# jinhojsk515/spmm

Measured on AMD Instinct MI355X. Metric: pretrain molecules/sec, higher is better.
Workload: dtype bf16; 1 GPU; SPMM pretrain step, text 12 layers (fusion at 6) + PV 6 layers, H=768, 12 heads, queue 36864, train mode (dropout 0.1), fwd+bwd+clip+AdamW+EMA; global_batch=128, seq_len=128, parallelism=dp1, schedule=eager launches on three HIP streams, packed text rows

## Files before the change

include/spmm_hip.h:

```cpp
#ifndef SPMM_HIP_H
#define SPMM_HIP_H

#include <stdint.h>

#ifdef __HIPCC__
#include <hip/hip_runtime.h>
typedef hipStream_t spmm_stream_t;
#else
typedef void* spmm_stream_t;
#endif

#ifdef __cplusplus
extern "C" {
#endif

int spmm_version(void);
const char* spmm_last_error(void);

#define SPMM_EPI_BF16 0
#define SPMM_EPI_GELU 1
#define SPMM_EPI_F32 2
#define SPMM_EPI_F32_ATOMIC 3
#define SPMM_EPI_GELU_GRAD 4
#define SPMM_EPI_F32_ACC 5
#define SPMM_EPI_GELU_DERIV 6
#define SPMM_EPI_MUL 7

#define SPMM_GEMM_AUTO 0
#define SPMM_GEMM_K128 1
#define SPMM_GEMM_K256x128 2
#define SPMM_GEMM_K256 3
#define SPMM_GEMM_K128PC 5
#define SPMM_GEMM_K256P8 8
#define SPMM_GEMM_K256P8_TILES 9
#define SPMM_GEMM_AUTO_TILES 16
int spmm_gemm_nt(const void* A, long lda, const void* W, long ldw, int M, int N, int K, int splits, const float* bias,
                 const float* div_ptr, float alpha, const void* R, long ldr, const void* G, long ldg, void* C, long ldc,
                 void* C2, long ldc2, int epi, float* colsum, int kernel, const int* M_dev, spmm_stream_t stream);
long spmm_gemm_tn_workspace_bytes(int M, int N, int K, int splits);
int spmm_gemm_tn_splits(int M, int N, int K, int kernel);
int spmm_gemm_tn(const void* A, long lda, const void* B, long ldb, int M, int N, int K, int splits, float alpha, float* C,
                 long ldc, float* workspace, int kernel, const int* M_dev, spmm_stream_t stream);
int spmm_gemm_tn_reduce(const float* ws, int ns, int N, int K, float* C, long ldc, spmm_stream_t stream);
int spmm_colsum_bf16(const void* x, long ld, int R, int C, float* out, const int* R_dev, spmm_stream_t stream);

int spmm_attn_fwd(const void* Q, long ldq, const void* K, long ldk, const void* V, long ldv, const int* kmask,
                  const int* kv_seq, const int* q_row0, const int* q_len, const int* kv_row0, const int* kv_len, void* O,
                  long ldo, float* LSE, int nseq, int nH, int Lq, int Lkv, int causal_from, int is_cross, float dropout_p,
                  const uint64_t* seed_ptr, uint64_t seed_salt, int q_off, int kv_off, spmm_stream_t stream);
int spmm_attn_bwd(const void* Q, long ldq, const void* K, long ldk, const void* V, long ldv, const int* kmask,
                  const int* kv_seq, const int* q_row0, const int* q_len, const int* kv_row0, const int* kv_len,
                  const void* O, long ldo, const float* LSE, const void* dO, long lddo, void* dQ,
                  long lddq, void* dK, long lddk, void* dV, long lddv, int nseq, int nH, int Lq, int Lkv, int causal_from,
                  int is_cross, float dropout_p, const uint64_t* seed_ptr, uint64_t seed_salt, int q_off, int kv_off, int d_mode,
                  float* Dbuf, spmm_stream_t stream);

int spmm_xattn_supported(int H, int nH, int Lq, int Lkv);
int spmm_xattn_pack_wo(const void* W, long ldw, void* out, int H, spmm_stream_t stream);
int spmm_xattn_fwd(const void* Q, long ldq, const void* K, long ldk, const void* V, long ldv, const int* kmask,
                   const int* kv_seq, const int* q_row0, const int* q_len, const int* kv_row0, const int* kv_len,
                   const void* WoF, const float* bo, const void* R, long ldr, const float* gamma, const float* beta, float eps,
                   void* Y, long ldy, void* Z, long ldz, float* mean, float* rstd, void* CTX, long ldc, float* LSE,
                   int nseq, int nH, int Lq, int Lkv, float attn_dropout_p, uint64_t salt_a, float hidden_dropout_p,
                   uint64_t salt_h, const uint64_t* seed_ptr, long row_base, spmm_stream_t stream);
int spmm_segment_sum_bf16(const void* src, const int* start, const int* list, void* out, int U, long W, spmm_stream_t stream);

int spmm_ln_fwd(const void* x, const void* res, const float* gamma, const float* beta, void* y, void* zout, float* mean,
                float* rstd, long rows, int H, float eps, float dropout_p, const uint64_t* seed_ptr, uint64_t salt,
                const int* rows_dev, spmm_stream_t stream);
int spmm_ln_fwd_r32(const void* x, const float* res32, const float* gamma, const float* beta, void* y, float* y32, void* zout,
                    float* mean, float* rstd, long rows, int H, float eps, float dropout_p, const uint64_t* seed_ptr,
// ... 90 lines not shown
```

spmm_amd/csrc/gemm.hip:

```cpp
#include "common.h"
#include "../../include/spmm_hip.h"

namespace {

constexpr int BM = 128, BN = 128, BK = 64;
constexpr int TILE_BYTES = BM * BK * 2;
constexpr int STAGE_BYTES = 2 * TILE_BYTES;

enum Epi { EPI_BF16 = 0, EPI_GELU = 1, EPI_F32 = 2, EPI_F32_ATOMIC = 3, EPI_GELU_GRAD = 4, EPI_F32_ACC = 5, EPI_GELU_DERIV = 6, EPI_MUL = 7 };
constexpr bool epi_is_bf16(int e) { return e == EPI_BF16 || e == EPI_GELU || e == EPI_GELU_GRAD || e == EPI_GELU_DERIV || e == EPI_MUL; }

struct GemmP {
  const bf16* A; long lda;
  const bf16* W; long ldw;
  int M, N, K;
  int ksplit;
  const float* bias;
  const float* div_ptr;
  float alpha;
  const bf16* R; long ldr;
  const bf16* G; long ldg;
  void* C; long ldc;
  bf16* C2; long ldc2;
  float* colsum;
  int order;
  const int* M_ptr;
};

#define GEMM_DYN_M(P)                                          \
  do {                                                         \
    if ((P).M_ptr) {                                           \
      const int m_ = *(P).M_ptr;                               \
      (P).M = m_ < (P).M ? (m_ > 0 ? m_ : 1) : (P).M;          \
    }                                                          \
  } while (0)

__device__ __forceinline__ void stage_tile_dma(const bf16* __restrict__ src, long ld, int row0, int nrows, int k0,
                                               char* lds_tile, int tid) {
#pragma unroll
  for (int c = 0; c < 4; ++c) {
    const int id = c * 256 + tid;
    const int row = id >> 3, ps = id & 7;
    const int ls = ps ^ ((row >> 1) & 7);
    int grow = row0 + row;
    grow = grow < nrows ? grow : nrows - 1;
    const bf16* g = src + (long)grow * ld + k0 + ls * 8;
    const int wave_base = __builtin_amdgcn_readfirstlane((c * 256 + (tid & ~63)) * 16);
    __builtin_amdgcn_global_load_lds((const GLOBAL_AS void*)g, (LDS_AS void*)(lds_tile + wave_base), 16, 0, 0);
  }
}

template <int EPI>
__device__ __forceinline__ void epi_convert(const GemmP& p, f32x16 (&acc)[2][2], char* t0, char* t1, int n_base, int lane) {
  float scale = p.alpha;
  if (p.div_ptr) scale /= *p.div_ptr;
#pragma unroll
  for (int ni = 0; ni < 2; ++ni)
#pragma unroll
    for (int mi = 0; mi < 2; ++mi) {
// ... 788 lines not shown
      if constexpr (HAS_EX && EPI == EPI_GELU_GRAD) {
        if (blk == 3) { P8_LOAD_EX(1); }
      } else if constexpr (HAS_EX) {
        if (h == 0) {
#pragma unroll
          for (int i_ = 2 * mi; i_ < 2 * mi + 2; ++i_) {
            long r_ = row0 + 64 + i_ * 8;
            if (!INTERIOR) r_ = r_ < p.M ? r_ : p.M - 1;
            P8_EX_LOAD1(i_, r_);
          }
        }
      }
    }
#undef P8_LOAD_EX
#undef P8_EX_LOAD1
  if constexpr (!GELU2) {
    if (p.colsum) {
#pragma unroll
      for (int e = 0; e < 8; ++e) {
        float t = cs[e];
        t += __shfl_xor(t, 8, 64);
        t += __shfl_xor(t, 16, 64);
        t += __shfl_xor(t, 32, 64);
        cs[e] = t;
      }
      if (lane < 8 && n_ok) {
#pragma unroll
        for (int e = 0; e < 8; ++e) atomicAdd(p.colsum + n + e, cs[e]);
      }
    }
  }
}

template <int EPI>
__global__ __launch_bounds__(512) void gemm_nt_p8_kernel(GemmP p) {
  extern __shared__ __attribute__((aligned(16))) char smem8[];
  const int tid = threadIdx.x, lane = tid & 63;
  const int wave = __builtin_amdgcn_readfirstlane(tid >> 6);
  const int wr = wave >> 2, wc = wave & 3;
  GEMM_DYN_M(p);
  const int ntm = (p.M + BM3 - 1) / BM3, ntn = (p.N + BN3 - 1) / BN3, nt = ntm * ntn;
  if ((int)blockIdx.x >= nt) return;
  const int nk = p.K / BK;

  f32x4 acc[2][4][4];
#define P8_ZERO()                                                              \
  _Pragma("unroll") for (int h_ = 0; h_ < 2; ++h_)                             \
  _Pragma("unroll") for (int i_ = 0; i_ < 4; ++i_)                             \
  _Pragma("unroll") for (int j_ = 0; j_ < 4; ++j_) acc[h_][i_][j_] = f32x4{0.f, 0.f, 0.f, 0.f}
  P8_ZERO();

  uint32_t offA[2][2], offW[2][2];
  const uint32_t ls16 = (uint32_t)(((tid & 7) ^ ((tid >> 4) & 7)) * 16);
  int m0, n0;
#define P8_TILE(VB)                                                                                           \
  do {                                                                                                        \
    const int b_ = (VB), q_ = nt >> 3, r_ = nt & 7, xcd_ = b_ & 7, i_ = b_ >> 3;                              \
    const int t_ = (xcd_ < r_ ? xcd_ * (q_ + 1) : r_ * (q_ + 1) + (xcd_ - r_) * q_) + i_;                     \
    int tm_, tn_;                                                                                             \
    tile_of(t_, ntm, ntn, p.order, tm_, tn_);                                                                 \
    m0 = tm_ * BM3; n0 = tn_ * BN3;                                                                           \
    _Pragma("unroll") for (int h_ = 0; h_ < 2; ++h_)                                                          \
    _Pragma("unroll") for (int j_ = 0; j_ < 2; ++j_) {                                                        \
      int row_ = m0 + j_ * 128 + h_ * 64 + (tid >> 3);                                                        \
      row_ = row_ < p.M ? row_ : p.M - 1;                     \
      offA[h_][j_] = (uint32_t)row_ * (uint32_t)(p.lda * 2) + ls16;                                                      \
      int col_ = n0 + (j_ * 2 + (tid >> 8)) * 64 + h_ * 32 + ((tid >> 3) & 31);                               \
      col_ = col_ < p.N ? col_ : p.N - 1;                                                                     \
      offW[h_][j_] = (uint32_t)col_ * (uint32_t)(p.ldw * 2) + ls16;                                                      \
    }                                                                                                         \
  } while (0)
  const char* gA = (const char*)p.A;
  const char* gW = (const char*)p.W;
  const uint32_t lds0 = (uint32_t)(uintptr_t)(LDS_AS char*)smem8;
#define P8_STG(GB, O, SLOT)                                                                                               \
  do {                                                                                                                    \
    const uint32_t d_ = lds0 + (SLOT) + wave * 1024;                                                                      \
    asm volatile("s_mov_b32 m0, %2\n\ts_nop 0\n\tglobal_load_lds_dwordx4 %0, %1" :: "v"((O)[0]), "s"(GB), "s"(d_) : "memory", "m0");          \
    asm volatile("s_mov_b32 m0, %2\n\ts_nop 0\n\tglobal_load_lds_dwordx4 %0, %1" :: "v"((O)[1]), "s"(GB), "s"(d_ + 8192) : "memory", "m0");   \
  } while (0)
#define P8_STG_A(H, BUF, KT) P8_STG((const char*)(gA + (size_t)(KT) * (BK * 2)), offA[H], (BUF) * P8_BUF + (H) * P8_HT)
#define P8_STG_W(H, BUF, KT) P8_STG((const char*)(gW + (size_t)(KT) * (BK * 2)), offW[H], (BUF) * P8_BUF + (2 + (H)) * P8_HT)
#define P8_PROLOGUE()                                                                        \
  do {                                                                                       \
    P8_STG_A(0, 0, 0); P8_STG_W(0, 0, 0); P8_STG_W(1, 0, 0); P8_STG_A(1, 0, 0);              \
    P8_STG_W(0, 1, 1); P8_STG_A(0, 1, 1); P8_STG_W(1, 1, 1);                                 \
  } while (0)

  uint32_t aad[2][2], wad[2][2];
  {
    const uint32_t sw = (uint32_t)((lane >> 1) & 7), r16 = (uint32_t)(lane & 15), q = (uint32_t)(lane >> 4);
#pragma unroll
    for (int kk = 0; kk < 2; ++kk) {
      const uint32_t slot = ((((uint32_t)kk * 4 + q) ^ sw) << 4);
      aad[0][kk] = lds0 + ((uint32_t)wr * 64 + r16) * 128 + slot;
      wad[0][kk] = lds0 + 2 * P8_HT + ((uint32_t)wc * 32 + r16) * 128 + slot;
      aad[1][kk] = aad[0][kk] + P8_BUF;
      wad[1][kk] = wad[0][kk] + P8_BUF;
    }
  }
  bf16x8 fa[4][2], fw0[2][2], fw1[2][2];
#define P8_RD_A(BUF, H)                                                                       \
// ... 27 lines not shown
#define P8_LGKM0() asm volatile("s_waitcnt lgkmcnt(0)" ::: "memory")
#define P8_COMPUTE(H, NH, FW)                    \
  do {                                           \
    P8_BAR();                                    \
    P8_LGKM0();                                  \
    P8_SB();                                     \
    __builtin_amdgcn_s_setprio(1);               \
    P8_MM(H, NH, FW);                            \
    __builtin_amdgcn_s_setprio(0);               \
    P8_SB();                                     \
    P8_BAR();                                    \
    P8_SB();                                     \
  } while (0)

#ifdef P8_PROFILE
  unsigned long long* prof = (unsigned long long*)p.colsum + (size_t)blockIdx.x * 16 * 8;
  p.colsum = nullptr;
  int prof_i = 0;
#define P8_STAMP(K) do { if (prof && tid == 0 && prof_i < 16) prof[prof_i * 8 + (K)] = __builtin_readcyclecounter(); } while (0)
#else
#define P8_STAMP(K) do { } while (0)
#endif
  int vb = blockIdx.x;
  bool pre = false;
  P8_TILE(vb);
  P8_PROLOGUE();
  asm volatile("s_waitcnt vmcnt(6)" ::: "memory");
  P8_BAR();
  P8_SB();
  if (wr == 1) P8_BAR();
  for (;;) {
    P8_STAMP(0);
    const int cm0 = m0, cn0 = n0;
    const int vbn = vb + (int)gridDim.x;
    const bool has_next = vbn < nt;
    const bool pre_next = has_next && cm0 + BM3 <= p.M && cn0 + BN3 <= p.N;
    for (int kt = 0; kt < nk; kt += 2) {
      const bool last = kt + 2 >= nk;
      const bool more = !last || has_next;
      int kn = kt + 2;
      P8_RD_W(0, 0, fw0); P8_SB(); P8_RD_A(0, 0);
      if (!(pre && kt == 0)) P8_STG_A(1, 1, kt + 1);
      asm volatile("s_waitcnt lgkmcnt(8)" ::: "memory");
      P8_COMPUTE(0, 0, fw0);
      if (last && has_next) { P8_TILE(vbn); kn = 0; }
      P8_RD_W(0, 1, fw1);
      if (more) P8_STG_W(0, 0, kn);
      P8_COMPUTE(0, 1, fw1);
      P8_RD_A(0, 1);
      if (more) P8_STG_A(0, 0, kn);
      P8_COMPUTE(1, 1, fw1);
      if (more) {
        P8_STG_W(1, 0, kn);
        if (pre && kt == 0) asm volatile("s_waitcnt vmcnt(22)" ::: "memory");
        else asm volatile("s_waitcnt vmcnt(6)" ::: "memory");
      } else {
        asm volatile("s_waitcnt vmcnt(0)" ::: "memory");
      }
      P8_COMPUTE(1, 0, fw0);
      P8_RD_W(1, 0, fw0); P8_SB(); P8_RD_A(1, 0);
      if (more) P8_STG_A(1, 0, kn);
      asm volatile("s_waitcnt lgkmcnt(8)" ::: "memory");
      P8_COMPUTE(0, 0, fw0);
      P8_RD_W(1, 1, fw1);
      if (more) P8_STG_W(0, 1, kn + 1);
      P8_COMPUTE(0, 1, fw1);
      P8_RD_A(1, 1);
      if (more) P8_STG_A(0, 1, kn + 1);
      P8_COMPUTE(1, 1, fw1);
      if (more) {
        P8_STG_W(1, 1, kn + 1);
        if (last && pre_next) {
          P8_STG_A(1, 1, kn + 1);
          asm volatile("s_waitcnt vmcnt(8)" ::: "memory");
        } else {
          asm volatile("s_waitcnt vmcnt(6)" ::: "memory");
        }
      }
      P8_COMPUTE(1, 0, fw0);
    }
    P8_STAMP(2);

    if (wr == 0) P8_BAR();
    P8_SB();
    {
      int lane_e = lane;
      asm volatile("" : "+v"(lane_e));
      GemmP q = p;
      asm volatile("" : "+s"(q.C), "+s"(q.ldc), "+s"(q.C2), "+s"(q.ldc2));
      asm volatile("" : "+s"(q.R), "+s"(q.ldr), "+s"(q.G), "+s"(q.ldg));
      asm volatile("" : "+s"(q.bias), "+s"(q.colsum), "+s"(q.div_ptr), "+s"(q.alpha), "+s"(q.M), "+s"(q.N));
      auto hook = [](int) {};
      const uint32_t xb = lds0 + P8_LDS + wave * 4096;
      const int mb = cm0 + wr * 128, nb = cn0 + wc * 64;
      const bool interior = cm0 + BM3 <= q.M && cn0 + BN3 <= q.N;
      if constexpr (EPI == EPI_GELU_GRAD || EPI == EPI_MUL) {
        if (interior) p8_epilogue_blocks<EPI, true, true>(q, acc, xb, mb, nb, lane_e, hook);
        else p8_epilogue_blocks<EPI, false, true>(q, acc, xb, mb, nb, lane_e, hook);
      } else if (EPI == EPI_BF16 && q.R != nullptr) {
        if (interior) p8_epilogue_blocks<EPI, true, true>(q, acc, xb, mb, nb, lane_e, hook);
        else p8_epilogue_blocks<EPI, false, true>(q, acc, xb, mb, nb, lane_e, hook);
      } else {
        if (interior) p8_epilogue_blocks<EPI, true, false>(q, acc, xb, mb, nb, lane_e, hook);
        else p8_epilogue_blocks<EPI, false, false>(q, acc, xb, mb, nb, lane_e, hook);
      }
    }
    P8_SB();
    if (wr == 1) P8_BAR();
    P8_STAMP(4);
#ifdef P8_PROFILE
    ++prof_i;
#endif
    if (!has_next) break;
    vb = vbn;
    pre = pre_next;
    P8_SB();
  }
  if (wr == 0) P8_BAR();
#undef P8_ZERO
#undef P8_STAMP
#undef P8_TILE
#undef P8_PROLOGUE
#undef P8_STG
#undef P8_STG_A
#undef P8_STG_W
#undef P8_RD_A
#undef P8_RD_W
#undef P8_MM
#undef P8_COMPUTE
#undef P8_BAR
#undef P8_SB
#undef P8_LGKM0
}

template <typename K>
int raise_lds(K kernel, int bytes, const char* what) {
  hipError_t e = hipFuncSetAttribute((const void*)kernel, hipFuncAttributeMaxDynamicSharedMemorySize, bytes);
  if (e != hipSuccess) {
    spmm_set_error("spmm_gemm_nt: cannot raise the dynamic LDS of %s to %d: %s", what, bytes, hipGetErrorString(e));
    return SPMM_ERR_LAUNCH;
  }
  return SPMM_OK;
}

template <int EPI>
int launch_p8_one(const GemmP& p, hipStream_t st, bool persist) {
  static const int rc = raise_lds(gemm_nt_p8_kernel<EPI>, P8_LDS + P8_XLDS, "the 8-phase kernel");
  if (rc != SPMM_OK) return rc;
  const int nt = ((p.M + BM3 - 1) / BM3) * ((p.N + BN3 - 1) / BN3);
  static const int ncu = [] { int dev = 0, n = 0; (void)hipGetDevice(&dev); (void)hipDeviceGetAttribute(&n, hipDeviceAttributeMultiprocessorCount, dev); return n > 0 ? n & ~7 : 256; }();
  dim3 grid(persist && nt > ncu ? ncu : nt);
  hipLaunchKernelGGL((gemm_nt_p8_kernel<EPI>), grid, dim3(512), P8_LDS + P8_XLDS, st, p);
  return SPMM_OK;
}
int launch_p8(int epi, const GemmP& p, hipStream_t st, bool persist) {
  switch (epi) {
    case EPI_BF16: return launch_p8_one<EPI_BF16>(p, st, persist);
    case EPI_GELU: return launch_p8_one<EPI_GELU>(p, st, persist);
    case EPI_GELU_GRAD: return launch_p8_one<EPI_GELU_GRAD>(p, st, persist);
    case EPI_GELU_DERIV: return launch_p8_one<EPI_GELU_DERIV>(p, st, persist);
    case EPI_MUL: return launch_p8_one<EPI_MUL>(p, st, persist);
    default: return -1;
  }
}

template <int EPI>
int launch_v3_one(const GemmP& p, hipStream_t st) {
  static const int rc = raise_lds(gemm_nt_v3_kernel<EPI>, LDS3_BYTES, "the 256x256 kernel");
  if (rc != SPMM_OK) return rc;
  dim3 grid(((p.M + BM3 - 1) / BM3) * ((p.N + BN3 - 1) / BN3));
  hipLaunchKernelGGL((gemm_nt_v3_kernel<EPI>), grid, dim3(512), LDS3_BYTES, st, p);
  return SPMM_OK;
}
int launch_v3(int epi, const GemmP& p, hipStream_t st) {
  switch (epi) {
    case EPI_BF16: return launch_v3_one<EPI_BF16>(p, st);
    case EPI_GELU: return launch_v3_one<EPI_GELU>(p, st);
    case EPI_GELU_GRAD: return launch_v3_one<EPI_GELU_GRAD>(p, st);
    case EPI_GELU_DERIV: return launch_v3_one<EPI_GELU_DERIV>(p, st);
    case EPI_MUL: return launch_v3_one<EPI_MUL>(p, st);
    default: return -1;
  }
}

// ... 46 lines not shown
    case EPI_F32_ATOMIC: hipLaunchKernelGGL((gemm_nt_kernel<EPI_F32_ATOMIC>), grid, dim3(256), 0, st, p); break;
    case EPI_GELU_GRAD: hipLaunchKernelGGL((gemm_nt_kernel<EPI_GELU_GRAD>), grid, dim3(256), 0, st, p); break;
    case EPI_F32_ACC: hipLaunchKernelGGL((gemm_nt_kernel<EPI_F32_ACC>), grid, dim3(256), 0, st, p); break;
    case EPI_GELU_DERIV: hipLaunchKernelGGL((gemm_nt_kernel<EPI_GELU_DERIV>), grid, dim3(256), 0, st, p); break;
    case EPI_MUL: hipLaunchKernelGGL((gemm_nt_kernel<EPI_MUL>), grid, dim3(256), 0, st, p); break;
    default: return -1;
  }
  return SPMM_OK;
}

inline bool is_bf16_epi(int epi) { return epi_is_bf16(epi); }
inline bool p8_ok(const GemmP& p, int epi) {
  return is_bf16_epi(epi) && p.K % 128 == 0 && p.N % 8 == 0 && (unsigned long)p.M * (unsigned long)p.lda * 2ul < (1ul << 32) &&
         (unsigned long)p.N * (unsigned long)p.ldw * 2ul < (1ul << 32);
}

int pick_tile(int M, int N, int epi) {
  const bool bf = is_bf16_epi(epi);
  if (M >= 6000) {
    const long t3 = (long)((M + 255) / 256) * ((N + 255) / 256);
    if (bf && t3 >= 96) return 3;
    return (epi != EPI_F32_ATOMIC) ? 2 : 1;
  }
  auto tiles = [&](int bm, int bn) { return (double)((M + bm - 1) / bm) * ((N + bn - 1) / bn); };
  auto fill = [](double t) { const double w = (double)(long)((t + 255) / 256); return t / (256.0 * w); };
  const double t3 = tiles(256, 256), t2 = tiles(256, 128), t1 = tiles(128, 128);
  const double s3 = bf ? 1.20 * fill(t3) : 0.0;
  const double s2 = (M >= 512 && epi != EPI_F32_ATOMIC) ? 0.85 * fill(t2) : 0.0;
  const double s1 = 0.80 * (t1 < 256 ? t1 / 256.0 : 1.0);
  if (s3 >= s2 && s3 >= s1) return 3;
  return s2 >= s1 ? 2 : 1;
}

}

extern "C" int spmm_gemm_nt(const void* A, long lda, const void* W, long ldw, int M, int N, int K, int splits,
                            const float* bias, const float* div_ptr, float alpha, const void* R, long ldr,
                            const void* G, long ldg, void* C, long ldc, void* C2, long ldc2, int epi, float* colsum,
                            int kernel, const int* M_dev, hipStream_t stream) {
  SPMM_CHECK_SHAPE(M > 0 && N > 0 && K > 0, "spmm_gemm_nt: empty problem M=%d N=%d K=%d", M, N, K);
  SPMM_CHECK_SHAPE(K % 64 == 0, "spmm_gemm_nt: K=%d must be a multiple of 64", K);
  SPMM_CHECK_SHAPE(N % 4 == 0, "spmm_gemm_nt: N=%d must be a multiple of 4", N);
  SPMM_CHECK_SHAPE(lda % 8 == 0 && ldw % 8 == 0, "spmm_gemm_nt: lda/ldw must be multiples of 8 elements");
  SPMM_CHECK_SHAPE(ldc % 4 == 0, "spmm_gemm_nt: ldc must be a multiple of 4");
  SPMM_CHECK_SHAPE(!is_bf16_epi(epi) || (ldc % 8 == 0 && (!R || ldr % 8 == 0) && (!G || ldg % 8 == 0) && (!C2 || ldc2 % 8 == 0) && (uintptr_t)C % 16 == 0),
                   "spmm_gemm_nt: bf16 outputs need 16-B aligned rows (ldc/ldr/ldg/ldc2 multiples of 8)");
  SPMM_CHECK_SHAPE(((uintptr_t)A % 16 == 0) && ((uintptr_t)W % 16 == 0), "spmm_gemm_nt: A/W must be 16-B aligned");
  SPMM_CHECK_SHAPE(epi >= EPI_BF16 && epi <= EPI_MUL, "spmm_gemm_nt: unknown epilogue %d", epi);
  if (splits < 1) splits = 1;
  SPMM_CHECK_SHAPE(splits == 1 || epi == EPI_F32_ATOMIC, "spmm_gemm_nt: split-K needs the atomic epilogue");
  SPMM_CHECK_SHAPE((epi != EPI_GELU_GRAD && epi != EPI_MUL) || G != nullptr, "spmm_gemm_nt: the GELU-grad / multiply epilogues need G");
  SPMM_CHECK_SHAPE(colsum == nullptr || epi == EPI_BF16 || epi == EPI_GELU_GRAD || epi == EPI_MUL, "spmm_gemm_nt: colsum is only fused into the bf16 / GELU-grad / multiply epilogues");
  int ksplit = ((K / 64 + splits - 1) / splits) * 64;
  splits = (K + ksplit - 1) / ksplit;
  GemmP p;
  p.A = (const bf16*)A; p.lda = lda; p.W = (const bf16*)W; p.ldw = ldw;
  p.M = M; p.N = N; p.K = K; p.ksplit = ksplit; p.bias = bias; p.div_ptr = div_ptr; p.alpha = alpha;
  p.R = (const bf16*)R; p.ldr = ldr; p.G = (const bf16*)G; p.ldg = ldg; p.C = C; p.ldc = ldc;
  p.C2 = (bf16*)C2; p.ldc2 = ldc2; p.colsum = colsum;
  p.M_ptr = nullptr;
  p.order = K > 1024 ? 0 : 2;

  int k = kernel == SPMM_GEMM_AUTO_TILES ? 0 : kernel;
  if (k == 0) {
    const int tile = splits > 1 ? 1 : pick_tile(M, N, epi);
    k = tile == 3 ? (p8_ok(p, epi) ? (kernel == SPMM_GEMM_AUTO_TILES ? 9 : 8) : 3) : tile;
    if (k == 2 && (epi == EPI_F32_ATOMIC || M < 512)) k = 1;
  }
  const bool pc_fits = (unsigned long)p.M * (unsigned long)p.lda * 2ul < (1ul << 32) && (unsigned long)p.N * (unsigned long)p.ldw * 2ul < (1ul << 32);
  const long t128 = (long)((M + BM - 1) / BM) * ((N + BN - 1) / BN) * splits;
  if (k == 1 && kernel != 1 && pc_fits && PC_AUTO && t128 <= 256 && ksplit >= 4 * BK) k = 5;
  SPMM_CHECK_SHAPE(k == 1 || k == 2 || k == 3 || k == 5 || k == 8 || k == 9, "spmm_gemm_nt: unknown kernel selector %d", kernel);
  SPMM_CHECK_SHAPE(k != 5 || pc_fits, "spmm_gemm_nt: kernel 5 addresses its operands with 32-bit byte offsets (< 4 GiB each)");
  SPMM_CHECK_SHAPE((k != 8 && k != 9) || p8_ok(p, epi), "spmm_gemm_nt: the 8-phase kernel needs a bf16-output epilogue, K %% 128 == 0, N %% 8 == 0 and operands < 4 GiB");
  SPMM_CHECK_SHAPE(k != 3 || is_bf16_epi(epi), "spmm_gemm_nt: the 256x256 kernel has bf16-output epilogues only");
  SPMM_CHECK_SHAPE(k != 2 || epi != EPI_F32_ATOMIC, "spmm_gemm_nt: the 256x128 kernel has no atomic epilogue");
  SPMM_CHECK_SHAPE(k == 1 || k == 5 || splits == 1, "spmm_gemm_nt: split-K runs on the 128x128 kernels only");
  p.M_ptr = M_dev;
  int rc;
  if (k == 8 || k == 9) rc = launch_p8(epi, p, stream, k == 8);
  else if (k == 3) rc = launch_v3(epi, p, stream);
  else if (k == 2) rc = launch_v2(epi, p, stream);
  else if (k == 5) rc = launch_pc(epi, p, dim3(((M + BM - 1) / BM) * ((N + BN - 1) / BN), 1, splits), stream);
  else rc = launch_v1(epi, p, dim3(((M + BM - 1) / BM) * ((N + BN - 1) / BN), 1, splits), stream);
  if (rc > 0) return rc;
  if (rc < 0) { spmm_set_error("spmm_gemm_nt: epilogue %d is not built for kernel %d", epi, k); return SPMM_ERR_UNSUPPORTED; }
  SPMM_LAUNCH_CHECK("spmm_gemm_nt");
  return SPMM_OK;
}
```

spmm_amd/engine.py:

```python
from __future__ import annotations

import contextlib
import functools
from dataclasses import dataclass
from typing import List, Optional

import torch

from . import ops, streams
from .config import BertConfig, SPMMConfig
from .options import EngineOptions
from .params import ParamStore

BF = torch.bfloat16
LOSS_MLM, LOSS_MPM, LOSS_ITA, LOSS_ITM = 0, 1, 2, 3


def _ceil(x, m):
    return (x + m - 1) // m * m


class KVSource:

    def __init__(self, kv: torch.Tensor, U: int, Lkv: int, row0=None, length=None, pack_idx=None):
# ... 60 lines not shown
        return self

    def attend(self, src: KVSource, idx: torch.Tensor) -> "Group":
        self.src, self.Lkv = src, src.Lkv
        self.kv_off = src.add(idx)
        self.kv_idx = idx.to(torch.int32)
        return self

    def cross_layout(self) -> dict:
        src = self.src
        return dict(kmask=self.kv_mask, kv_seq=self.kv_idx, q_row0=self.q_row0, q_len=self.q_len,
                    kv_row0=None if src is None else src.row0, kv_len=None if src is None else src.len)


@dataclass
class Batch:
    groups: List[Group]
    rows_dev: Optional[torch.Tensor] = None

    def __iter__(self):
        return iter(self.groups)

    def __len__(self):
        return len(self.groups)


STREAM_TOKENS_MAX = 49152


class Engine:
    def __init__(self, cfg: SPMMConfig, params: ParamStore, device, options: Optional[EngineOptions] = None):
        self.cfg, self.P, self.dev = cfg, params, device
        self.opt = options if options is not None else EngineOptions.from_env()
        if torch.device(device).type == "cuda":
            from ._lib import bind_device
            bind_device(torch.device(device).index if torch.device(device).index is not None else torch.cuda.current_device())
        f32 = dict(dtype=torch.float32, device=device)
        self.alpha = torch.zeros(1, **f32)
        self.lr = torch.zeros(1, **f32)
        self.gscale = torch.ones(4, **f32)
        self.step_zero = torch.zeros(16, dtype=torch.int32, device=device)
        self.losses = self.step_zero[0:8].view(torch.float32)
        self.loss_scratch = torch.zeros(8, **f32)
        rank = torch.distributed.get_rank() if (torch.distributed.is_available() and torch.distributed.is_initialized()) else 0
        self.seed_rank_offset = rank * 0x9E3779B97F4A7C15 % (1 << 62)
        self.seed = torch.full((1,), (0x5DEECE66D + self.seed_rank_offset) % (1 << 62), dtype=torch.int64, device=device)
        self.nan_flag = self.step_zero[9:10]
        self.icount = torch.zeros(4, dtype=torch.int32, device=device)
        self.dtemp_ita = self.step_zero[8:9].view(torch.float32)
        self.train_mode = True
        self.hint_bad = self.step_zero[10:11]
        self.pack_text = self.opt.pack_text
        self.layer_done_cb = None
        self.multi_stream = self.opt.multi_stream
        self.wgrad_async = self.opt.wgrad_stream and self.multi_stream
        self._one_stream = False
        dist_ = torch.distributed
        will_exchange = dist_.is_available() and dist_.is_initialized() and (dist_.get_world_size() > 1 or self.opt.force_dist)
        self._one_side = bool(will_exchange and self.opt.dp_four_streams)
        if self.multi_stream and torch.device(device).type == "cuda" and not ops._DRY_RUN and not will_exchange:
            streams.bind_in_order(device, ("side0", "side1", "wgrad"))
        self.force_one_stream = False
        self._wg_stream, self._wg_pending, self._wg_keep = None, False, []
        self._salt = 0
        self._off_path_ok, self._pre_bwd = False, None
        self._xattn_checked = self._xattn_off = False
# ... 497 lines not shown
```

spmm_amd/ops.py:

```python
import ctypes
import os

import torch

from ._lib import lib

EPI_BF16, EPI_GELU, EPI_F32, EPI_F32_ATOMIC, EPI_GELU_GRAD, EPI_F32_ACC, EPI_GELU_DERIV, EPI_MUL = range(8)
BF16 = torch.bfloat16


_DRY_RUN = False
_dry_log = []


def _p(t):
    return None if t is None else ctypes.c_void_p(t.data_ptr())


def _st():
    if _DRY_RUN:
        return None
    return ctypes.c_void_p(torch.cuda.current_stream().cuda_stream)


# ... 19 lines not shown
            raise TypeError(f"{name}: argument {i} = {a!r} is not a {t.__name__}") from e
        if t is ctypes.c_void_p and not (a is None or isinstance(a, (ctypes.c_void_p, int))):
            raise TypeError(f"{name}: argument {i} must be a pointer, got {type(a)}")
    _dry_log.append(name)


def _row_stride(t):
    assert t.dim() == 2 and (t.stride(1) == 1 or t.shape[1] == 1), (t.shape, t.stride())
    return t.stride(0)


GEMM_AUTO, GEMM_AUTO_TILES = 0, 16
_nt_auto = GEMM_AUTO


class nt_tiles_per_workgroup:

    def __init__(self, on=True):
        self.on = on

    def __enter__(self):
        global _nt_auto
        self._prev = _nt_auto
        if self.on:
            _nt_auto = GEMM_AUTO_TILES
        return self

    def __exit__(self, *exc):
        global _nt_auto
        _nt_auto = self._prev
        return False


def gemm_nt(A, W, C, *, bias=None, epi=EPI_BF16, R=None, G=None, C2=None, alpha=1.0, div=None, splits=1, K=None, colsum=None, kernel=0,
            M_dev=None):
    if kernel == 0:
        kernel = _nt_auto
    M, Ka = A.shape
    N = W.shape[0]
    K = Ka if K is None else K
    assert A.dtype == BF16 and W.dtype == BF16 and W.shape[1] >= K and C.shape[0] >= M and C.shape[1] >= N
    if epi in (EPI_BF16, EPI_GELU, EPI_GELU_GRAD, EPI_GELU_DERIV, EPI_MUL):
        assert C.dtype == BF16
    else:
        assert C.dtype == torch.float32
    _call("spmm_gemm_nt", _p(A), _row_stride(A), _p(W), _row_stride(W), M, N, K, splits, _p(bias), _p(div),
               float(alpha), _p(R), 0 if R is None else _row_stride(R), _p(G), 0 if G is None else _row_stride(G),
               _p(C), _row_stride(C), _p(C2), 0 if C2 is None else _row_stride(C2), epi, _p(colsum), int(kernel), _p(M_dev), _st())
    return C


def gemm_tn(A, B, C, *, alpha=1.0, splits=None, kernel=0, M_dev=None):
    M, N = A.shape
    K = B.shape[1]
    assert A.dtype == BF16 and B.dtype == BF16 and C.dtype == torch.float32 and B.shape[0] == M and tuple(C.shape) == (N, K)
    if splits is None:
        splits = 1 if _DRY_RUN else lib().cdll.spmm_gemm_tn_splits(M, N, K, int(kernel))
    ws = torch.empty(splits * N * K, dtype=torch.float32, device=C.device) if splits > 1 else None
    _call("spmm_gemm_tn", _p(A), _row_stride(A), _p(B), _row_stride(B), M, N, K, splits, float(alpha), _p(C), _row_stride(C), _p(ws),
          int(kernel), _p(M_dev), _st())
    return C


def colsum_bf16(x, out, *, R_dev=None):
    R, C = x.shape
    _call("spmm_colsum_bf16", _p(x), _row_stride(x), R, C, _p(out), _p(R_dev), _st())
    return out


def attn_fwd(Q, K, V, O, lse, *, nseq, nH, Lq, Lkv, kmask=None, causal_from=None, is_cross=False, dropout_p=0.0,
             seed=None, salt=0, kv_seq=None, q_row0=None, q_len=None, kv_row0=None, kv_len=None, q_off=0, kv_off=0):
    cf = nseq if causal_from is None else causal_from
    _call("spmm_attn_fwd", _p(Q), _row_stride(Q), _p(K), _row_stride(K), _p(V), _row_stride(V), _p(kmask), _p(kv_seq), _p(q_row0),
               _p(q_len), _p(kv_row0), _p(kv_len), _p(O),
               _row_stride(O), _p(lse), nseq, nH, Lq, Lkv, cf, int(is_cross), float(dropout_p), _p(seed), salt, int(q_off), int(kv_off), _st())
    return O


def attn_bwd(Q, K, V, O, lse, dO, dQ, dK, dV, *, nseq, nH, Lq, Lkv, kmask=None, causal_from=None, is_cross=False,
             dropout_p=0.0, seed=None, salt=0, kv_seq=None, q_row0=None, q_len=None, kv_row0=None, kv_len=None, q_off=0, kv_off=0,
             d_mode=0, dbuf=None):
# ... 434 lines not shown
```

spmm_amd/options.py:

```python
from __future__ import annotations

import dataclasses
import os
from dataclasses import dataclass

_ENV = {
    "pack_text": ("SPMM_PACK_TEXT", lambda s: s != "0"),
    "cls_only_top": ("SPMM_CLS_ONLY_TOP", lambda s: s != "0"),
    "multi_stream": ("SPMM_STREAMS", lambda s: s != "1"),
    "wgrad_stream": ("SPMM_WGRAD_STREAM", lambda s: s != "0"),
    "pv_wgrad_inline": ("SPMM_PV_WGRAD_INLINE", int),
    "ln_from_y": ("SPMM_LN_FROM_Y", lambda s: s != "0"),
    "resid_fp32": ("SPMM_RESID_FP32", lambda s: s == "1"),
    "fused_xattn": ("SPMM_FUSED_XATTN", lambda s: {"0": "off", "1": "all"}.get(s, s)),
    "grad_overlap": ("SPMM_GRAD_OVERLAP", lambda s: s != "0"),
    "grad_wire": ("SPMM_GRAD_WIRE", str),
    "nt_under_comm": ("SPMM_NT_UNDER_COMM", str),
    "force_dist": ("SPMM_FORCE_DIST", lambda s: s == "1"),
    "dp_four_streams": ("SPMM_DP_FOUR_STREAMS", lambda s: s != "0"),
    "probe_streams": ("SPMM_PROBE_STREAMS", lambda s: s != "0"),
    "schedule_check": ("SPMM_SCHEDULE_CHECK", lambda s: s != "0"),
}


@dataclass
class EngineOptions:
    pack_text: bool = True
    cls_only_top: bool = True
    multi_stream: bool = True
    wgrad_stream: bool = True
    pv_wgrad_inline: int = 4
    ln_from_y: bool = True
    fused_xattn: str = "nograd"
    resid_fp32: bool = False
    grad_overlap: bool = True
    grad_wire: str = "fp32"
    nt_under_comm: str = "auto"
    force_dist: bool = False
    dp_four_streams: bool = True
    schedule_check: bool = True
    probe_streams: bool = False

    @classmethod
    def from_env(cls, **overrides) -> "EngineOptions":
        kw = {}
        for field, (var, parse) in _ENV.items():
            if var in os.environ:
                kw[field] = parse(os.environ[var])
        kw.update(overrides)
        o = cls(**kw)
        if isinstance(o.fused_xattn, bool):
            o.fused_xattn = "all" if o.fused_xattn else "off"
        if o.fused_xattn not in ("off", "nograd", "all"):
            raise ValueError(f"fused_xattn must be off, nograd or all, not {o.fused_xattn!r}")
        if o.grad_wire not in ("fp32", "bf16"):
            raise ValueError(f"grad_wire must be fp32 or bf16, not {o.grad_wire!r}")
        if o.nt_under_comm not in ("tiles", "persistent", "auto"):
            raise ValueError(f"nt_under_comm must be tiles, persistent or auto, not {o.nt_under_comm!r}")
        return o

    def replace(self, **kw) -> "EngineOptions":
        return dataclasses.replace(self, **kw)
```

Measured before the change: 2485 molecules/s.

## Split-K the partial final wave of the persistent 8-phase NT GEMM

Tiles left over after the last full wave of 256 blocks in the persistent 8-phase NT GEMM are now split along K into up to four slices. Each slice writes its fp32 partial accumulators to a workspace slab, and the last block to arrive, found through an atomic ticket counter, sums the slabs and runs the epilogue. This is meant to fill the idle compute units during the tail wave. In exchange it adds workspace traffic, an atomic handshake with fences, and a per-stream workspace allocation on the Python side, and it disables next-tile prefetch for the split items.

Result: slower. 2455 molecules/s (-1.2%).

```diff
diff --git a/include/spmm_hip.h b/include/spmm_hip.h
--- a/include/spmm_hip.h
+++ b/include/spmm_hip.h
@@ -37,6 +37,12 @@
 int spmm_gemm_nt(const void* A, long lda, const void* W, long ldw, int M, int N, int K, int splits, const float* bias,
                  const float* div_ptr, float alpha, const void* R, long ldr, const void* G, long ldg, void* C, long ldc,
                  void* C2, long ldc2, int epi, float* colsum, int kernel, const int* M_dev, spmm_stream_t stream);
+long spmm_gemm_nt_tail_workspace_bytes(int M, int N, int K, int epi, int kernel, int has_M_dev);
+int spmm_gemm_nt_ws(const void* A, long lda, const void* W, long ldw, int M, int N, int K, int splits, const float* bias,
+                    const float* div_ptr, float alpha, const void* R, long ldr, const void* G, long ldg, void* C, long ldc,
+                    void* C2, long ldc2, int epi, float* colsum, int kernel, const int* M_dev, void* workspace, long workspace_bytes,
+                    spmm_stream_t stream);
+int spmm_gemm_nt_tail_plan(int M, int N, int K, int item, int* out);
 long spmm_gemm_tn_workspace_bytes(int M, int N, int K, int splits);
 int spmm_gemm_tn_splits(int M, int N, int K, int kernel);
 int spmm_gemm_tn(const void* A, long lda, const void* B, long ldb, int M, int N, int K, int splits, float alpha, float* C,
diff --git a/spmm_amd/csrc/gemm.hip b/spmm_amd/csrc/gemm.hip
--- a/spmm_amd/csrc/gemm.hip
+++ b/spmm_amd/csrc/gemm.hip
@@ -25,6 +25,8 @@
   float* colsum;
   int order;
   const int* M_ptr;
+  float* tail_ws;
+  unsigned* tail_cnt;
 };
 
 #define GEMM_DYN_M(P)                                          \
@@ -879,6 +881,115 @@
   }
 }
 
+constexpr int P8_G = 256;
+#ifndef P8_TAIL_SMAX
+#define P8_TAIL_SMAX 4
+#endif
+#ifndef P8_TAIL_MINK
+#define P8_TAIL_MINK 8
+#endif
+#ifndef P8_TAIL_MAXR
+#define P8_TAIL_MAXR 128
+#endif
+static_assert(P8_TAIL_SMAX >= 1 && P8_TAIL_SMAX <= 8 && P8_TAIL_MINK >= 2 && P8_TAIL_MINK % 2 == 0 && P8_TAIL_MAXR <= P8_G / 2, "tail constants");
+constexpr long P8_TAIL_CNT_BYTES = 4096;
+constexpr long P8_TAIL_SLAB_BYTES = 256l * 256 * 4;
+struct P8Tail { int full, r, s; };
+struct P8Item { int vb, slice, ns, kt0, nk; };
+__host__ __device__ inline P8Tail p8_tail_plan(int nt, int nk, bool on) {
+  P8Tail t;
+  t.full = nt / P8_G * P8_G; t.r = nt - t.full; t.s = 1;
+  if (on && t.r > 0 && t.r <= P8_TAIL_MAXR) {
+    int s = P8_G / t.r;
+    s = s < P8_TAIL_SMAX ? s : P8_TAIL_SMAX;
+    s = s < nk / P8_TAIL_MINK ? s : nk / P8_TAIL_MINK;
+    t.s = s > 1 ? s : 1;
+  }
+  return t;
+}
+__host__ __device__ inline int p8_tail_items(const P8Tail& t) { return t.full + t.r * t.s; }
+__host__ __device__ inline int p8_tail_k0(int nk, int s, int i) { return (nk / 2) * i / s * 2; }
+__host__ __device__ inline P8Item p8_tail_item(const P8Tail& t, int nk, int w) {
+  P8Item it;
+  it.vb = w; it.slice = 0; it.ns = 1; it.kt0 = 0; it.nk = nk;
+  if (t.s > 1 && w >= t.full) {
+    const int j = w - t.full;
+    it.slice = j / t.r; it.vb = t.full + j % t.r; it.ns = t.s;
+    it.kt0 = p8_tail_k0(nk, t.s, it.slice);
+    it.nk = p8_tail_k0(nk, t.s, it.slice + 1) - it.kt0;
+  }
+  return it;
+}
+
+__device__ __forceinline__ void p8_gst(GLOBAL_AS f32x4* dst, const f32x4& v) {
+  asm volatile("global_store_dwordx4 %0, %1, off" :: "v"(dst), "v"(v) : "memory");
+}
+__device__ __forceinline__ void p8_gld(f32x4& d, const GLOBAL_AS f32x4* src) {
+  asm volatile("global_load_dwordx4 %0, %1, off" : "=v"(d) : "v"(src) : "memory");
+}
+template <bool FIRST>
+__device__ __forceinline__ void p8_tail_add(f32x4 (&acc)[2][4][4], const GLOBAL_AS f32x4* src) {
+#pragma unroll
+  for (int h = 0; h < 2; ++h)
+#pragma unroll
+    for (int mh = 0; mh < 2; ++mh) {
+      f32x4 t[2][4];
+#pragma unroll
+      for (int m2 = 0; m2 < 2; ++m2)
+#pragma unroll
+        for (int ni = 0; ni < 4; ++ni) p8_gld(t[m2][ni], src + ((h * 4 + mh * 2 + m2) * 4 + ni) * 64);
+      asm volatile("s_waitcnt vmcnt(0)" : "+v"(t[0][0]), "+v"(t[0][1]), "+v"(t[0][2]), "+v"(t[0][3]), "+v"(t[1][0]), "+v"(t[1][1]), "+v"(t[1][2]), "+v"(t[1][3]) :: "memory");
+#pragma unroll
+      for (int m2 = 0; m2 < 2; ++m2)
+#pragma unroll
+        for (int ni = 0; ni < 4; ++ni) {
+          if (FIRST) acc[h][mh * 2 + m2][ni] = t[m2][ni];
+          else acc[h][mh * 2 + m2][ni] += t[m2][ni];
+        }
+    }
+}
+__device__ __forceinline__ bool p8_tail_arrive(float* ws, unsigned* cnt, f32x4 (&acc)[2][4][4], int slot, int ns, int slice, uint32_t flag_lds,
+                                               int wave) {
+  const int lane = (int)__builtin_amdgcn_mbcnt_hi(~0u, __builtin_amdgcn_mbcnt_lo(~0u, 0u));
+  typedef GLOBAL_AS f32x4 gf32x4;
+  gf32x4* slab = (gf32x4*)ws + ((size_t)(slot * ns + slice) << 14) + wave * (32 * 64) + lane;
+#pragma unroll
+  for (int h = 0; h < 2; ++h)
+#pragma unroll
+    for (int mi = 0; mi < 4; ++mi)
+#pragma unroll
+      for (int ni = 0; ni < 4; ++ni) p8_gst(slab + ((h * 4 + mi) * 4 + ni) * 64, acc[h][mi][ni]);
+  asm volatile("s_waitcnt vmcnt(0)" ::: "memory");
+  __builtin_amdgcn_s_barrier();
+  __builtin_amdgcn_sched_barrier(0);
+  if (wave == 0 && lane == 0) {
+    __builtin_amdgcn_fence(__ATOMIC_RELEASE, "agent");
+    asm volatile("s_waitcnt vmcnt(0)" ::: "memory");
+    const unsigned ticket = __hip_atomic_fetch_add(cnt + slot, 1u, __ATOMIC_RELAXED, __HIP_MEMORY_SCOPE_AGENT);
+    const uint32_t last = ticket == (unsigned)(ns - 1) ? 1u : 0u;
+    if (last) {
+      __builtin_amdgcn_fence(__ATOMIC_ACQUIRE, "agent");
+      asm volatile("s_waitcnt vmcnt(0)" ::: "memory");
+      __hip_atomic_store(cnt + slot, 0u, __ATOMIC_RELAXED, __HIP_MEMORY_SCOPE_AGENT);
+    }
+    asm volatile("ds_write_b32 %0, %1\n\ts_waitcnt lgkmcnt(0)" :: "v"(flag_lds), "v"(last) : "memory");
+  }
+  __builtin_amdgcn_sched_barrier(0);
+  __builtin_amdgcn_s_barrier();
+  uint32_t flag;
+  asm volatile("ds_read_b32 %0, %1\n\ts_waitcnt lgkmcnt(0)" : "=v"(flag) : "v"(flag_lds) : "memory");
+  __builtin_amdgcn_s_barrier();
+  __builtin_amdgcn_sched_barrier(0);
+  if (!__builtin_amdgcn_readfirstlane(flag)) return false;
+  const gf32x4* src = (const gf32x4*)ws + ((size_t)(slot * ns) << 14) + wave * (32 * 64) + lane;
+  p8_tail_add<true>(acc, src);
+  for (int i = 1; i < ns; ++i) {
+    src += 1 << 14;
+    p8_tail_add<false>(acc, src);
+  }
+  return true;
+}
+
 template <int EPI>
 __global__ __launch_bounds__(512) void gemm_nt_p8_kernel(GemmP p) {
   extern __shared__ __attribute__((aligned(16))) char smem8[];
@@ -887,8 +998,9 @@
   const int wr = wave >> 2, wc = wave & 3;
   GEMM_DYN_M(p);
   const int ntm = (p.M + BM3 - 1) / BM3, ntn = (p.N + BN3 - 1) / BN3, nt = ntm * ntn;
-  if ((int)blockIdx.x >= nt) return;
   const int nk = p.K / BK;
+  const int nitems = __builtin_amdgcn_readfirstlane(p8_tail_items(p8_tail_plan(nt, nk, p.tail_ws != nullptr)));
+  if ((int)blockIdx.x >= nitems) return;
 
   f32x4 acc[2][4][4];
 #define P8_ZERO()                                                              \
@@ -900,9 +1012,17 @@
   uint32_t offA[2][2], offW[2][2];
   const uint32_t ls16 = (uint32_t)(((tid & 7) ^ ((tid >> 4) & 7)) * 16);
   int m0, n0;
+  int item_nk, item_tail;
 #define P8_TILE(VB)                                                                                           \
   do {                                                                                                        \
-    const int b_ = (VB), q_ = nt >> 3, r_ = nt & 7, xcd_ = b_ & 7, i_ = b_ >> 3;                              \
+    int nt_ = nt;                                                                                             \
+    asm volatile("" : "+s"(nt_));                                                                             \
+    const P8Tail tp_ = p8_tail_plan(nt_, nk, p.tail_ws != nullptr);                                           \
+    const P8Item it_ = p8_tail_item(tp_, nk, (VB));                                                           \
+    item_nk = __builtin_amdgcn_readfirstlane(it_.nk);                                                         \
+    item_tail = __builtin_amdgcn_readfirstlane(it_.ns > 1 ? (it_.vb - tp_.full) << 8 | it_.slice << 4 | it_.ns : 0); \
+    const uint32_t k0_ = (uint32_t)__builtin_amdgcn_readfirstlane(it_.kt0 * (BK * 2));                        \
+    const int b_ = __builtin_amdgcn_readfirstlane(it_.vb), q_ = nt >> 3, r_ = nt & 7, xcd_ = b_ & 7, i_ = b_ >> 3; \
     const int t_ = (xcd_ < r_ ? xcd_ * (q_ + 1) : r_ * (q_ + 1) + (xcd_ - r_) * q_) + i_;                     \
     int tm_, tn_;                                                                                             \
     tile_of(t_, ntm, ntn, p.order, tm_, tn_);                                                                 \
@@ -911,10 +1031,10 @@
     _Pragma("unroll") for (int j_ = 0; j_ < 2; ++j_) {                                                        \
       int row_ = m0 + j_ * 128 + h_ * 64 + (tid >> 3);                                                        \
       row_ = row_ < p.M ? row_ : p.M - 1;                     \
-      offA[h_][j_] = (uint32_t)row_ * (uint32_t)(p.lda * 2) + ls16;                                                      \
+      offA[h_][j_] = (uint32_t)row_ * (uint32_t)(p.lda * 2) + ls16 + k0_;                                                    \
       int col_ = n0 + (j_ * 2 + (tid >> 8)) * 64 + h_ * 32 + ((tid >> 3) & 31);                               \
       col_ = col_ < p.N ? col_ : p.N - 1;                                                                     \
-      offW[h_][j_] = (uint32_t)col_ * (uint32_t)(p.ldw * 2) + ls16;                                                      \
+      offW[h_][j_] = (uint32_t)col_ * (uint32_t)(p.ldw * 2) + ls16 + k0_;                                                    \
     }                                                                                                         \
   } while (0)
   const char* gA = (const char*)p.A;
@@ -1008,11 +1128,12 @@
   for (;;) {
     P8_STAMP(0);
     const int cm0 = m0, cn0 = n0;
+    const int nkc = item_nk, cur_tail = item_tail;
     const int vbn = vb + (int)gridDim.x;
-    const bool has_next = vbn < nt;
-    const bool pre_next = has_next && cm0 + BM3 <= p.M && cn0 + BN3 <= p.N;
-    for (int kt = 0; kt < nk; kt += 2) {
-      const bool last = kt + 2 >= nk;
+    const bool has_next = vbn < nitems;
+    const bool pre_next = has_next && cm0 + BM3 <= p.M && cn0 + BN3 <= p.N && cur_tail == 0;
+    for (int kt = 0; kt < nkc; kt += 2) {
+      const bool last = kt + 2 >= nkc;
       const bool more = !last || has_next;
       int kn = kt + 2;
       P8_RD_W(0, 0, fw0); P8_SB(); P8_RD_A(0, 0);
@@ -1059,8 +1180,17 @@
 
     if (wr == 0) P8_BAR();
     P8_SB();
-    {
-      int lane_e = lane;
+    bool owner = true;
+    if (cur_tail != 0) {
+      float* ws_ = p.tail_ws;
+      unsigned* cnt_ = p.tail_cnt;
+      asm volatile("" : "+s"(ws_), "+s"(cnt_));
+      owner = p8_tail_arrive(ws_, cnt_, acc, cur_tail >> 8, cur_tail & 15, (cur_tail >> 4) & 15, lds0 + P8_LDS, wave);
+      if (!owner && has_next) P8_ZERO();
+    }
+    P8_SB();
+    if (owner) {
+      int lane_e = (int)__builtin_amdgcn_mbcnt_hi(~0u, __builtin_amdgcn_mbcnt_lo(~0u, 0u));
       asm volatile("" : "+v"(lane_e));
       GemmP q = p;
       asm volatile("" : "+s"(q.C), "+s"(q.ldc), "+s"(q.C2), "+s"(q.ldc2));
@@ -1124,8 +1254,10 @@
   static const int rc = raise_lds(gemm_nt_p8_kernel<EPI>, P8_LDS + P8_XLDS, "the 8-phase kernel");
   if (rc != SPMM_OK) return rc;
   const int nt = ((p.M + BM3 - 1) / BM3) * ((p.N + BN3 - 1) / BN3);
+  int items = nt;
+  if (p.tail_ws) items = p.M_ptr ? (nt / P8_G + 1) * P8_G : p8_tail_items(p8_tail_plan(nt, p.K / BK, true));
   static const int ncu = [] { int dev = 0, n = 0; (void)hipGetDevice(&dev); (void)hipDeviceGetAttribute(&n, hipDeviceAttributeMultiprocessorCount, dev); return n > 0 ? n & ~7 : 256; }();
-  dim3 grid(persist && nt > ncu ? ncu : nt);
+  dim3 grid(persist && items > ncu ? ncu : items);
   hipLaunchKernelGGL((gemm_nt_p8_kernel<EPI>), grid, dim3(512), P8_LDS + P8_XLDS, st, p);
   return SPMM_OK;
 }
@@ -1238,12 +1370,20 @@
   return s2 >= s1 ? 2 : 1;
 }
 
-}
-
-extern "C" int spmm_gemm_nt(const void* A, long lda, const void* W, long ldw, int M, int N, int K, int splits,
-                            const float* bias, const float* div_ptr, float alpha, const void* R, long ldr,
-                            const void* G, long ldg, void* C, long ldc, void* C2, long ldc2, int epi, float* colsum,
-                            int kernel, const int* M_dev, hipStream_t stream) {
+long tail_bytes(int M, int N, int K, int epi, int kernel, bool has_M_dev) {
+  if (M <= 0 || N <= 0 || K <= 0 || (kernel != SPMM_GEMM_AUTO && kernel != SPMM_GEMM_AUTO_TILES)) return 0;
+  GemmP p;
+  p.M = M; p.N = N; p.K = K; p.lda = K; p.ldw = K;
+  if (pick_tile(M, N, epi) != 3 || !p8_ok(p, epi)) return 0;
+  if (has_M_dev) return K / BK / P8_TAIL_MINK >= 2 ? P8_TAIL_CNT_BYTES + P8_G * P8_TAIL_SLAB_BYTES : 0;
+  const P8Tail t = p8_tail_plan(((M + BM3 - 1) / BM3) * ((N + BN3 - 1) / BN3), K / BK, true);
+  return t.s > 1 ? P8_TAIL_CNT_BYTES + (long)t.r * t.s * P8_TAIL_SLAB_BYTES : 0;
+}
+
+int gemm_nt_impl(const void* A, long lda, const void* W, long ldw, int M, int N, int K, int splits,
+                 const float* bias, const float* div_ptr, float alpha, const void* R, long ldr,
+                 const void* G, long ldg, void* C, long ldc, void* C2, long ldc2, int epi, float* colsum,
+                 int kernel, const int* M_dev, void* workspace, long workspace_bytes, hipStream_t stream) {
   SPMM_CHECK_SHAPE(M > 0 && N > 0 && K > 0, "spmm_gemm_nt: empty problem M=%d N=%d K=%d", M, N, K);
   SPMM_CHECK_SHAPE(K % 64 == 0, "spmm_gemm_nt: K=%d must be a multiple of 64", K);
   SPMM_CHECK_SHAPE(N % 4 == 0, "spmm_gemm_nt: N=%d must be a multiple of 4", N);
@@ -1265,6 +1405,7 @@
   p.R = (const bf16*)R; p.ldr = ldr; p.G = (const bf16*)G; p.ldg = ldg; p.C = C; p.ldc = ldc;
   p.C2 = (bf16*)C2; p.ldc2 = ldc2; p.colsum = colsum;
   p.M_ptr = nullptr;
+  p.tail_ws = nullptr; p.tail_cnt = nullptr;
   p.order = K > 1024 ? 0 : 2;
 
   int k = kernel == SPMM_GEMM_AUTO_TILES ? 0 : kernel;
@@ -1283,6 +1424,11 @@
   SPMM_CHECK_SHAPE(k != 2 || epi != EPI_F32_ATOMIC, "spmm_gemm_nt: the 256x128 kernel has no atomic epilogue");
   SPMM_CHECK_SHAPE(k == 1 || k == 5 || splits == 1, "spmm_gemm_nt: split-K runs on the 128x128 kernels only");
   p.M_ptr = M_dev;
+  if ((k == 8 || k == 9) && workspace) {
+    const long need = tail_bytes(M, N, K, epi, kernel, M_dev != nullptr);
+    SPMM_CHECK_SHAPE(workspace_bytes >= need && (uintptr_t)workspace % 16 == 0, "spmm_gemm_nt_ws: workspace of %ld bytes, %ld needed (16-B aligned)", workspace_bytes, need);
+    if (need > 0) { p.tail_cnt = (unsigned*)workspace; p.tail_ws = (float*)((char*)workspace + P8_TAIL_CNT_BYTES); }
+  }
   int rc;
   if (k == 8 || k == 9) rc = launch_p8(epi, p, stream, k == 8);
   else if (k == 3) rc = launch_v3(epi, p, stream);
@@ -1294,3 +1440,36 @@
   SPMM_LAUNCH_CHECK("spmm_gemm_nt");
   return SPMM_OK;
 }
+
+}
+
+extern "C" int spmm_gemm_nt(const void* A, long lda, const void* W, long ldw, int M, int N, int K, int splits,
+                            const float* bias, const float* div_ptr, float alpha, const void* R, long ldr,
+                            const void* G, long ldg, void* C, long ldc, void* C2, long ldc2, int epi, float* colsum,
+                            int kernel, const int* M_dev, hipStream_t stream) {
+  return gemm_nt_impl(A, lda, W, ldw, M, N, K, splits, bias, div_ptr, alpha, R, ldr, G, ldg, C, ldc, C2, ldc2, epi, colsum, kernel, M_dev,
+                      nullptr, 0, stream);
+}
+
+extern "C" long spmm_gemm_nt_tail_workspace_bytes(int M, int N, int K, int epi, int kernel, int has_M_dev) {
+  return tail_bytes(M, N, K, epi, kernel, has_M_dev != 0);
+}
+
+extern "C" int spmm_gemm_nt_ws(const void* A, long lda, const void* W, long ldw, int M, int N, int K, int splits,
+                               const float* bias, const float* div_ptr, float alpha, const void* R, long ldr,
+                               const void* G, long ldg, void* C, long ldc, void* C2, long ldc2, int epi, float* colsum,
+                               int kernel, const int* M_dev, void* workspace, long workspace_bytes, hipStream_t stream) {
+  return gemm_nt_impl(A, lda, W, ldw, M, N, K, splits, bias, div_ptr, alpha, R, ldr, G, ldg, C, ldc, C2, ldc2, epi, colsum, kernel, M_dev,
+                      workspace, workspace_bytes, stream);
+}
+
+extern "C" int spmm_gemm_nt_tail_plan(int M, int N, int K, int item, int* out) {
+  const int nt = ((M + BM3 - 1) / BM3) * ((N + BN3 - 1) / BN3), nk = K / BK;
+  const P8Tail t = p8_tail_plan(nt, nk, true);
+  out[0] = nt; out[1] = t.full; out[2] = t.r; out[3] = t.s;
+  if (item >= 0) {
+    const P8Item it = p8_tail_item(t, nk, item);
+    out[4] = it.vb; out[5] = it.slice; out[6] = it.kt0; out[7] = it.nk;
+  }
+  return p8_tail_items(t);
+}
diff --git a/spmm_amd/engine.py b/spmm_amd/engine.py
--- a/spmm_amd/engine.py
+++ b/spmm_amd/engine.py
@@ -116,6 +116,7 @@
     def __init__(self, cfg: SPMMConfig, params: ParamStore, device, options: Optional[EngineOptions] = None):
         self.cfg, self.P, self.dev = cfg, params, device
         self.opt = options if options is not None else EngineOptions.from_env()
+        ops.set_nt_tail_split(self.opt.nt_tail_split)
         if torch.device(device).type == "cuda":
             from ._lib import bind_device
             bind_device(torch.device(device).index if torch.device(device).index is not None else torch.cuda.current_device())
diff --git a/spmm_amd/ops.py b/spmm_amd/ops.py
--- a/spmm_amd/ops.py
+++ b/spmm_amd/ops.py
@@ -75,6 +75,32 @@
         return False
 
 
+_nt_tail = True
+_nt_tail_bytes = {}
+_nt_tail_ws = {}
+
+
+def set_nt_tail_split(on):
+    global _nt_tail
+    _nt_tail = bool(on)
+
+
+def _nt_tail_workspace(M, N, K, epi, kernel, has_M_dev, device):
+    if not _nt_tail or _DRY_RUN or kernel not in (GEMM_AUTO, GEMM_AUTO_TILES):
+        return None
+    key = (M, N, K, epi, kernel, has_M_dev)
+    n = _nt_tail_bytes.get(key)
+    if n is None:
+        n = _nt_tail_bytes[key] = lib().cdll.spmm_gemm_nt_tail_workspace_bytes(M, N, K, epi, kernel, int(has_M_dev))
+    if n == 0:
+        return None
+    skey = (device.index, torch.cuda.current_stream().cuda_stream)
+    ws = _nt_tail_ws.get(skey)
+    if ws is None or ws.numel() < n:
+        ws = _nt_tail_ws[skey] = torch.zeros(n, dtype=torch.uint8, device=device)
+    return ws
+
+
 def gemm_nt(A, W, C, *, bias=None, epi=EPI_BF16, R=None, G=None, C2=None, alpha=1.0, div=None, splits=1, K=None, colsum=None, kernel=0,
             M_dev=None):
     if kernel == 0:
@@ -87,9 +113,14 @@
         assert C.dtype == BF16
     else:
         assert C.dtype == torch.float32
-    _call("spmm_gemm_nt", _p(A), _row_stride(A), _p(W), _row_stride(W), M, N, K, splits, _p(bias), _p(div),
-               float(alpha), _p(R), 0 if R is None else _row_stride(R), _p(G), 0 if G is None else _row_stride(G),
-               _p(C), _row_stride(C), _p(C2), 0 if C2 is None else _row_stride(C2), epi, _p(colsum), int(kernel), _p(M_dev), _st())
+    args = (_p(A), _row_stride(A), _p(W), _row_stride(W), M, N, K, splits, _p(bias), _p(div),
+            float(alpha), _p(R), 0 if R is None else _row_stride(R), _p(G), 0 if G is None else _row_stride(G),
+            _p(C), _row_stride(C), _p(C2), 0 if C2 is None else _row_stride(C2), epi, _p(colsum), int(kernel), _p(M_dev))
+    ws = _nt_tail_workspace(M, N, K, epi, int(kernel), M_dev is not None, A.device) if splits == 1 else None
+    if ws is None:
+        _call("spmm_gemm_nt", *args, _st())
+    else:
+        _call("spmm_gemm_nt_ws", *args, _p(ws), ws.numel(), _st())
     return C
 
 
diff --git a/spmm_amd/options.py b/spmm_amd/options.py
--- a/spmm_amd/options.py
+++ b/spmm_amd/options.py
@@ -12,6 +12,7 @@
     "pv_wgrad_inline": ("SPMM_PV_WGRAD_INLINE", int),
     "ln_from_y": ("SPMM_LN_FROM_Y", lambda s: s != "0"),
     "resid_fp32": ("SPMM_RESID_FP32", lambda s: s == "1"),
+    "nt_tail_split": ("SPMM_NT_TAIL_SPLIT", lambda s: s != "0"),
     "fused_xattn": ("SPMM_FUSED_XATTN", lambda s: {"0": "off", "1": "all"}.get(s, s)),
     "grad_overlap": ("SPMM_GRAD_OVERLAP", lambda s: s != "0"),
     "grad_wire": ("SPMM_GRAD_WIRE", str),
@@ -31,6 +32,7 @@
     wgrad_stream: bool = True
     pv_wgrad_inline: int = 4
     ln_from_y: bool = True
+    nt_tail_split: bool = True
     fused_xattn: str = "nograd"
     resid_fp32: bool = False
     grad_overlap: bool = True
```
